# YukeWang96/QGTC_PPoPP22

Measured on AMD Instinct MI355X. Metric: effective bit-GEMM TOPS (2*M*K*N/t), 1-bit A x 1-bit X, M=K=4096, N=64, higher is better.
Workload: dtype fp4 (E2M1 codes of bit planes on MFMA, exact f32 sums); 1 GPU; bitMM2Bit 4096x4096x64 a=1 w=1 ob=1 (BASELINE.json configs[1], 2_7c shape); inputs=seeded Bernoulli(0.5) adjacency, uniform w-bit features, packed, resident in HBM, parallelism=replica-per-GPU x1, no data-path collective, engine=auto, issue=eager

## Files before the change

qgtc_ppopp22_amd/csrc/bitmm_fp4_one.hip.h:

```cpp
#pragma once

namespace {

constexpr int ONE_WAVES = 8;
constexpr int ONE_MAX_K = 4 * 128 * ONE_WAVES;

template <int NP>
__device__ __forceinline__ void one_expand(const u32x4 (&pl)[NP], int digit, uint32_t (&ops)[4][4], int (&scale)[4]) {
    if constexpr (NP == 1) {
#pragma unroll
        for (int t = 0; t < 4; t++) {
            const uint32_t wd = pl[0][t];
            ops[0][t] = wd & 0x11111111u;
            ops[1][t] = wd & 0x22222222u;
            ops[2][t] = wd & 0x44444444u;
            ops[3][t] = (wd >> 3) & 0x11111111u;
        }
        scale[0] = 128; scale[1] = 127; scale[2] = 126; scale[3] = 128;
    } else {
#pragma unroll
        for (int t = 0; t < 4; t++) {
            const uint32_t w0 = pl[2 * digit][t], w1 = 2 * digit + 1 < NP ? pl[(2 * digit + 1) % NP][t] : 0u;
            uint32_t ev = (w0 & 0x55555555u) | ((w1 & 0x55555555u) << 1), od = ((w0 >> 1) & 0x55555555u) | (w1 & 0xaaaaaaaau);
            asm("" : "+v"(ev), "+v"(od));
            ops[0][t] = ev & 0x33333333u;
            ops[1][t] = od & 0x33333333u;
            ops[2][t] = (ev >> 2) & 0x33333333u;
            ops[3][t] = (od >> 2) & 0x33333333u;
        }
#pragma unroll
        for (int s = 0; s < 4; s++) scale[s] = 128 + 2 * digit;
    }
}

template <int NA, int NW, int MODE, int RF, int CF>
__global__ __launch_bounds__(64 * ONE_WAVES) void k_bitmm_fp4_one(
    const uint32_t *__restrict__ Xp, const uint32_t *__restrict__ Wp, void *__restrict__ outp, uint32_t x_bytes,
    uint32_t w_bytes, uint32_t out_bytes, int M, int K, int N, int w_lines,
    uint32_t cfg ) {
    static_assert(NA >= 1 && NA <= 8 && NW >= 1 && NW <= 8, "plane capacities");
    static_assert(MODE != 1 || RF == 2, "cols-layout words need whole 32-row tiles");
    constexpr int NF = RF * CF;
    constexpr int NDA = (NA + 1) / 2, NDW = (NW + 1) / 2;
    constexpr bool SWAP = MODE != 1;
    __shared__ __attribute__((aligned(16))) f32x4 part[ONE_WAVES][NF][64];
    const int tid = threadIdx.x, lane = tid & 63;
    const int wv = __builtin_amdgcn_readfirstlane(tid >> 6);
    const int li = lane & 15, g = lane >> 4;
    const int kq = (K + 127) >> 7;
    const int m0 = blockIdx.x * (16 * RF), n0 = blockIdx.y * (16 * CF);
    const int a = cfg & 255u, w = (cfg >> 8) & 255u, ob = (cfg >> 16) & 255u;
    const bool zero_skip = ((cfg >> 24) & 1u) != 0u;
    const int nwv = min(ONE_WAVES, (kq + 3) >> 2);
    const bool worker = 4 * wv < kq;

#ifdef QGTC_STAMPS
    unsigned long long st_[8] = {0, 0, 0, 0, 0, 0, 0, 0};
#define ONE_STAMP(i) st_[i] = __builtin_amdgcn_s_memtime()
#else
#define ONE_STAMP(i) do { } while (0)
#endif
    ONE_STAMP(0);
    f32x4 acc[RF][CF];
    u32x4 xr[RF][NA], wr[CF][NW];
    {
        const uint32_t row_bytes = static_cast<uint32_t>(kq) * 16u;
        const int q = 4 * wv + g;
        const uint32_t ko = static_cast<uint32_t>(q) * 16u;
        const bool q_ok = q < kq;
        const __amdgpu_buffer_rsrc_t rx = __builtin_amdgcn_make_buffer_rsrc(const_cast<uint32_t *>(Xp), 0, static_cast<int>(x_bytes), 0x00020000);
        const __amdgpu_buffer_rsrc_t rw = __builtin_amdgcn_make_buffer_rsrc(const_cast<uint32_t *>(Wp), 0, static_cast<int>(w_bytes), 0x00020000);
        const uint32_t x_plane = static_cast<uint32_t>(pad8(M)) * row_bytes, w_plane = static_cast<uint32_t>(w_lines) * row_bytes;
#pragma unroll
        for (int i = 0; i < RF; i++) {
            const int m = m0 + 16 * i + li;
            uint32_t off = __umul24(static_cast<uint32_t>(m), row_bytes) + ko;
#ifdef QGTC_ABL
            if (cfg & (1u << 28)) off = static_cast<uint32_t>(lane) * 16u;
#endif
#pragma unroll
            for (int p = 0; p < NA; p++)
                xr[i][p] = __builtin_amdgcn_raw_buffer_load_b128(rx, (q_ok && m < M && p < a) ? off + static_cast<uint32_t>(p) * x_plane : 0xffffffffu, 0, 0);
        }
#pragma unroll
        for (int j = 0; j < CF; j++) {
            const int n = n0 + 16 * j + li;
            uint32_t off = __umul24(static_cast<uint32_t>(n), row_bytes) + ko;
#ifdef QGTC_ABL
            if (cfg & (1u << 29)) off = static_cast<uint32_t>(lane) * 16u;
#endif
#pragma unroll
            for (int p = 0; p < NW; p++)
                wr[j][p] = __builtin_amdgcn_raw_buffer_load_b128(rw, (q_ok && n < N && p < w) ? off + static_cast<uint32_t>(p) * w_plane : 0xffffffffu, 0, 0);
        }
    }
    if (worker) {
        ONE_STAMP(1);
        uint32_t any = 0u;
#pragma unroll
        for (int i = 0; i < RF; i++)
#pragma unroll
            for (int p = 0; p < NA; p++) any |= (xr[i][p].x | xr[i][p].y) | (xr[i][p].z | xr[i][p].w);
        const bool mult = !zero_skip || __ballot(any != 0u) != 0ull;
        if (!mult) {
#pragma unroll
            for (int i = 0; i < RF; i++)
#pragma unroll
                for (int j = 0; j < CF; j++) acc[i][j] = f32x4{0.0f, 0.0f, 0.0f, 0.0f};
        } else {
#ifdef QGTC_STAGGER_EXP
            if ((cfg & (1u << 30)) && wv >= 4) __builtin_amdgcn_s_sleep(6);
            if ((cfg & (1u << 31))) { if (wv >= 4) __builtin_amdgcn_s_setprio(0); else __builtin_amdgcn_s_setprio(2); }
            if ((cfg & (1u << 27)) && wv >= 4) __builtin_amdgcn_s_sleep(12);
#endif
            uint32_t xo[RF][NDA][4][4], wo[4][4];
            int xs[RF][NDA][4], ws[4];
#pragma unroll
            for (int i = 0; i < RF; i++)
#pragma unroll
                for (int da = 0; da < NDA; da++) one_expand<NA>(xr[i], da, xo[i][da], xs[i][da]);
#pragma unroll
            for (int j = 0; j < CF; j++)
#pragma unroll
                for (int dw = 0; dw < NDW; dw++) {
                    one_expand<NW>(wr[j], dw, wo, ws);
#pragma unroll
                    for (int s = 0; s < 4; s++) {
                        const i32x4 b4 = {static_cast<int>(wo[s][0]), static_cast<int>(wo[s][1]), static_cast<int>(wo[s][2]), static_cast<int>(wo[s][3])};
                        const i32x8 b8 = __builtin_shufflevector(b4, b4, 0, 1, 2, 3, -1, -1, -1, -1);
#pragma unroll
                        for (int i = 0; i < RF; i++)
#pragma unroll
                            for (int da = 0; da < NDA; da++) {
                                const i32x4 a4 = {static_cast<int>(xo[i][da][s][0]), static_cast<int>(xo[i][da][s][1]), static_cast<int>(xo[i][da][s][2]), static_cast<int>(xo[i][da][s][3])};
                                const i32x8 a8 = __builtin_shufflevector(a4, a4, 0, 1, 2, 3, -1, -1, -1, -1);
                                const f32x4 c = (dw == 0 && s == 0 && da == 0) ? f32x4{0.0f, 0.0f, 0.0f, 0.0f} : acc[i][j];
                                if (SWAP) acc[i][j] = __builtin_amdgcn_mfma_scale_f32_16x16x128_f8f6f4(b8, a8, c, 4, 4, 0, ws[s], 0, xs[i][da][s]);
                                else acc[i][j] = __builtin_amdgcn_mfma_scale_f32_16x16x128_f8f6f4(a8, b8, c, 4, 4, 0, xs[i][da][s], 0, ws[s]);
                            }
                    }
                }
        }
#ifdef QGTC_STAMPS
        asm volatile("" : "+v"(acc[0][0]));
#endif
        ONE_STAMP(2);
#pragma unroll
        for (int i = 0; i < RF; i++)
#pragma unroll
            for (int j = 0; j < CF; j++) part[wv][i * CF + j][lane] = acc[i][j];
    }
    int n_valid = 0;
    uint32_t vnib = 0u, oplane_bytes = 0u, o_off = 0xffffffffu, sh = 0u;
    bool store = false;
    const __amdgpu_buffer_rsrc_t ro = __builtin_amdgcn_make_buffer_rsrc(outp, 0, static_cast<int>(out_bytes), 0x00020000);
    if (wv < NF) {
        const int fi = wv / CF, fj = wv % CF;
        const int line = (SWAP ? m0 + 16 * fi : n0 + 16 * fj) + li;
        const int elem0 = (SWAP ? n0 + 16 * fj : m0 + 16 * fi) + 4 * g;
        const int line_lim = SWAP ? M : N, elem_lim = SWAP ? N : M;
        n_valid = line < line_lim ? min(max(elem_lim - elem0, 0), 4) : 0;
        vnib = (0xf0u >> n_valid) & 0xfu;
        const int pitch = SWAP ? step128(N) * 4 : step128(M) * 4;
        const int n_lines = SWAP ? pad8(M) : pad128(N);
        oplane_bytes = static_cast<uint32_t>(n_lines) * static_cast<uint32_t>(pitch) * 4u;
        const int frag0 = SWAP ? n0 + 16 * fj : m0 + 16 * fi;
        const int word = frag0 >> 5;
        o_off = MODE == 2 ? (static_cast<uint32_t>(line) * static_cast<uint32_t>(N) + static_cast<uint32_t>(elem0)) * 4u
                          : (static_cast<uint32_t>(line) * static_cast<uint32_t>(pitch) + static_cast<uint32_t>(word)) * 4u + ((frag0 & 16) ? 0u : 2u);
        store = MODE == 2 ? line < M : (g == 0 && line < n_lines && word < pitch);
        if (!store) o_off = 0xffffffffu;
        sh = 12u - 4u * static_cast<uint32_t>(g);
        asm volatile("" : "+v"(o_off) : "v"(vnib), "v"(sh), "s"(oplane_bytes));
    }
    ONE_STAMP(3);
    __syncthreads();
    ONE_STAMP(4);

    if (wv >= NF) {
        uint32_t *out = static_cast<uint32_t *>(outp);
        const int t = tid - 64 * NF, nt = 64 * (ONE_WAVES - NF);
        if (MODE == 0) {
            const int rows_pad = pad8(M), row_words = step128(N) * 4;
            const int w_next = (n0 + 16 * CF + 31) >> 5;
            if (static_cast<int>(blockIdx.y) == (N + 16 * CF - 1) / (16 * CF) - 1 && w_next < row_words) {
                const int nx = row_words - w_next;
                for (int e = t; e < ob * 16 * RF * nx; e += nt) {
                    const int x = e % nx, r = (e / nx) % (16 * RF), p = e / (nx * 16 * RF);
                    if (m0 + r < rows_pad) out[(static_cast<size_t>(p) * rows_pad + m0 + r) * row_words + w_next + x] = 0u;
                }
            }
        } else if (MODE == 1) {
            const int lines = pad128(N), line_words = step128(M) * 4;
            const size_t oplane = static_cast<size_t>(lines) * line_words;
            const bool last_m = static_cast<int>(blockIdx.x) == (M + 16 * RF - 1) / (16 * RF) - 1, last_n = static_cast<int>(blockIdx.y) == (N + 16 * CF - 1) / (16 * CF) - 1;
            const int word1 = m0 >> 5, w_core1 = min(line_words, word1 + 1);
            if (last_m && w_core1 < line_words) {
                for (int e = t; e < ob * 16 * CF; e += nt) {
                    const int line = n0 + e % (16 * CF), p = e / (16 * CF);
                    if (line < lines)
                        for (int wi = w_core1; wi < line_words; wi++) out[p * oplane + static_cast<size_t>(line) * line_words + wi] = 0u;
                }
            }
            if (last_n && n0 + 16 * CF < lines) {
                const int nl = lines - (n0 + 16 * CF), w_end = last_m ? line_words : w_core1;
                for (int e = t; e < ob * nl; e += nt) {
                    const int line = n0 + 16 * CF + e % nl, p = e / nl;
                    for (int wi = word1; wi < w_end; wi++) out[p * oplane + static_cast<size_t>(line) * line_words + wi] = 0u;
                }
            }
        }
        return;
    }

    f32x4 sum;
    if (nwv == ONE_WAVES) {
        f32x4 pv[ONE_WAVES];
#ifdef QGTC_ABL_HALFRED
#pragma unroll
        for (int p = 0; p < ONE_WAVES / 2; p++) pv[p] = part[p][wv][lane];
        sum = (pv[0] + pv[1]) + (pv[2] + pv[3]);
#else
#pragma unroll
        for (int p = 0; p < ONE_WAVES; p++) pv[p] = part[p][wv][lane];
        sum = ((pv[0] + pv[1]) + (pv[2] + pv[3])) + ((pv[4] + pv[5]) + (pv[6] + pv[7]));
#endif
    } else {
        sum = part[0][wv][lane];
        for (int p = 1; p < nwv; p++) sum += part[p][wv][lane];
    }
    ONE_STAMP(5);
    if (MODE == 2) {
        const u32x4 v4 = __builtin_bit_cast(u32x4, sum);
        if (n_valid == 4) {
            __builtin_amdgcn_raw_buffer_store_b128(v4, ro, o_off, 0, 0);
        } else {
            if (n_valid >= 2) __builtin_amdgcn_raw_buffer_store_b64(u32x2{v4.x, v4.y}, ro, o_off, 0, 0);
            if (n_valid == 3) __builtin_amdgcn_raw_buffer_store_b32(v4.z, ro, o_off + 8u, 0, 0);
            if (n_valid == 1) __builtin_amdgcn_raw_buffer_store_b32(v4.x, ro, o_off, 0, 0);
        }
    } else {
        const int maxi = 1 << ob;
        uint32_t P = 0u;
#pragma unroll
        for (int e = 0; e < 4; e++) {
            const int c = static_cast<int>(sum[e]);
            P = (P << 8) | (static_cast<uint32_t>(c > maxi ? maxi - 1 : c) & 255u);
        }
        int qhi[4];
        if (ob > 8) {
#pragma unroll
            for (int e = 0; e < 4; e++) {
                const int c = static_cast<int>(sum[e]);
                qhi[e] = c > maxi ? maxi - 1 : c;
            }
        }
        for (int p = 0; p < ob; p++, o_off += store ? oplane_bytes : 0u) {
            uint32_t t;
            if (p < 8) t = (P >> p) & 0x01010101u;
            else t = ((qhi[0] >> p) & 1) << 24 | ((qhi[1] >> p) & 1) << 16 | ((qhi[2] >> p) & 1) << 8 | ((qhi[3] >> p) & 1);
            uint32_t x = (((t >> 21) | (t >> 14)) | ((t >> 7) | t)) & vnib;
            x <<= sh;
            const auto s16 = __builtin_amdgcn_permlane16_swap(x, x, false, false);
            x = s16[0] | s16[1];
            x = or_with_partner_half(x);
            __builtin_amdgcn_raw_buffer_store_b16(static_cast<unsigned short>(x), ro, o_off, 0, 0);
        }
    }
#ifdef QGTC_STAMPS
    ONE_STAMP(6);
    if (tid == 0 && blockIdx.y == 0 && blockIdx.x < 1024)
        for (int i = 0; i < 8; i++) g_stamps[blockIdx.x * 16 + i] = st_[i];
#endif
#undef ONE_STAMP
}

}
```

Baseline: 738.2 TOPS.

## Simplify load addressing, move pad zeroing into output waves, early-exit idle waves

Load offsets are now built from a per-lane base plus wave-uniform scalar terms, and the per-row bounds checks on X/W loads are dropped, so address math is cheaper. The zero-skip path writes zeros straight into the shared partials, and the accumulator is scoped to the multiply branch. Non-output waves now sync and return earlier. MODE 0 padding zeroing moves from the idle waves into the output waves as per-lane b32 stores placed beside the reduction loads. The cost is that correctness now depends on padded rows (M, N) staying in bounds, and MODE 0 padding now rides on the store waves.

Result: slower. 632.1 TOPS (-14.4%).

```diff
diff --git a/qgtc_ppopp22_amd/csrc/bitmm_fp4_one.hip.h b/qgtc_ppopp22_amd/csrc/bitmm_fp4_one.hip.h
--- a/qgtc_ppopp22_amd/csrc/bitmm_fp4_one.hip.h
+++ b/qgtc_ppopp22_amd/csrc/bitmm_fp4_one.hip.h
@@ -61,37 +61,37 @@
 #define ONE_STAMP(i) do { } while (0)
 #endif
     ONE_STAMP(0);
-    f32x4 acc[RF][CF];
     u32x4 xr[RF][NA], wr[CF][NW];
     {
         const uint32_t row_bytes = static_cast<uint32_t>(kq) * 16u;
-        const int q = 4 * wv + g;
-        const uint32_t ko = static_cast<uint32_t>(q) * 16u;
-        const bool q_ok = q < kq;
+        const uint32_t lo = __umul24(static_cast<uint32_t>(li), row_bytes) + static_cast<uint32_t>(g) * 16u;
+        const bool q_ok = (lane & 48) < 16 * (kq - 4 * wv);
         const __amdgpu_buffer_rsrc_t rx = __builtin_amdgcn_make_buffer_rsrc(const_cast<uint32_t *>(Xp), 0, static_cast<int>(x_bytes), 0x00020000);
         const __amdgpu_buffer_rsrc_t rw = __builtin_amdgcn_make_buffer_rsrc(const_cast<uint32_t *>(Wp), 0, static_cast<int>(w_bytes), 0x00020000);
         const uint32_t x_plane = static_cast<uint32_t>(pad8(M)) * row_bytes, w_plane = static_cast<uint32_t>(w_lines) * row_bytes;
+        const uint32_t ux = static_cast<uint32_t>(m0) * row_bytes + 64u * static_cast<uint32_t>(wv);
+        const uint32_t uw = static_cast<uint32_t>(n0) * row_bytes + 64u * static_cast<uint32_t>(wv);
 #pragma unroll
         for (int i = 0; i < RF; i++) {
-            const int m = m0 + 16 * i + li;
-            uint32_t off = __umul24(static_cast<uint32_t>(m), row_bytes) + ko;
+#pragma unroll
+            for (int p = 0; p < NA; p++) {
+                uint32_t off = lo + (ux + static_cast<uint32_t>(16 * i) * row_bytes + static_cast<uint32_t>(p) * x_plane);
 #ifdef QGTC_ABL
-            if (cfg & (1u << 28)) off = static_cast<uint32_t>(lane) * 16u;
-#endif
-#pragma unroll
-            for (int p = 0; p < NA; p++)
-                xr[i][p] = __builtin_amdgcn_raw_buffer_load_b128(rx, (q_ok && m < M && p < a) ? off + static_cast<uint32_t>(p) * x_plane : 0xffffffffu, 0, 0);
+                if (cfg & (1u << 28)) off = static_cast<uint32_t>(lane) * 16u;
+#endif
+                xr[i][p] = __builtin_amdgcn_raw_buffer_load_b128(rx, (q_ok && (p == 0 || p < a)) ? off : 0xffffffffu, 0, 0);
+            }
         }
 #pragma unroll
         for (int j = 0; j < CF; j++) {
-            const int n = n0 + 16 * j + li;
-            uint32_t off = __umul24(static_cast<uint32_t>(n), row_bytes) + ko;
+#pragma unroll
+            for (int p = 0; p < NW; p++) {
+                uint32_t off = lo + (uw + static_cast<uint32_t>(16 * j) * row_bytes + static_cast<uint32_t>(p) * w_plane);
 #ifdef QGTC_ABL
-            if (cfg & (1u << 29)) off = static_cast<uint32_t>(lane) * 16u;
-#endif
-#pragma unroll
-            for (int p = 0; p < NW; p++)
-                wr[j][p] = __builtin_amdgcn_raw_buffer_load_b128(rw, (q_ok && n < N && p < w) ? off + static_cast<uint32_t>(p) * w_plane : 0xffffffffu, 0, 0);
+                if (cfg & (1u << 29)) off = static_cast<uint32_t>(lane) * 16u;
+#endif
+                wr[j][p] = __builtin_amdgcn_raw_buffer_load_b128(rw, (p == 0 || p < w) ? off : 0xffffffffu, 0, 0);
+            }
         }
     }
     if (worker) {
@@ -102,12 +102,14 @@
 #pragma unroll
             for (int p = 0; p < NA; p++) any |= (xr[i][p].x | xr[i][p].y) | (xr[i][p].z | xr[i][p].w);
         const bool mult = !zero_skip || __ballot(any != 0u) != 0ull;
-        if (!mult) {
-#pragma unroll
-            for (int i = 0; i < RF; i++)
-#pragma unroll
-                for (int j = 0; j < CF; j++) acc[i][j] = f32x4{0.0f, 0.0f, 0.0f, 0.0f};
+        if (__builtin_expect(!mult, 0)) {
+            f32x4 z = {0.0f, 0.0f, 0.0f, 0.0f};
+            asm volatile("" : "+v"(z));
+#pragma unroll
+            for (int f = 0; f < NF; f++) part[wv][f][lane] = z;
+            asm volatile("" ::: "memory");
         } else {
+            f32x4 acc[RF][CF];
 #ifdef QGTC_STAGGER_EXP
             if ((cfg & (1u << 30)) && wv >= 4) __builtin_amdgcn_s_sleep(6);
             if ((cfg & (1u << 31))) { if (wv >= 4) __builtin_amdgcn_s_setprio(0); else __builtin_amdgcn_s_setprio(2); }
@@ -140,21 +142,50 @@
                             }
                     }
                 }
-        }
 #ifdef QGTC_STAMPS
-        asm volatile("" : "+v"(acc[0][0]));
-#endif
-        ONE_STAMP(2);
-#pragma unroll
-        for (int i = 0; i < RF; i++)
-#pragma unroll
-            for (int j = 0; j < CF; j++) part[wv][i * CF + j][lane] = acc[i][j];
-    }
-    int n_valid = 0;
-    uint32_t vnib = 0u, oplane_bytes = 0u, o_off = 0xffffffffu, sh = 0u;
-    bool store = false;
+            asm volatile("" : "+v"(acc[0][0]));
+#endif
+            ONE_STAMP(2);
+#pragma unroll
+            for (int i = 0; i < RF; i++)
+#pragma unroll
+                for (int j = 0; j < CF; j++) part[wv][i * CF + j][lane] = acc[i][j];
+        }
+    }
+    if (wv >= NF) {
+        __syncthreads();
+        if (MODE == 1) {
+            uint32_t *out = static_cast<uint32_t *>(outp);
+            const int t = tid - 64 * NF, nt = 64 * (ONE_WAVES - NF);
+            const int lines = pad128(N), line_words = step128(M) * 4;
+            const size_t oplane = static_cast<size_t>(lines) * line_words;
+            const bool last_m = static_cast<int>(blockIdx.x) == (M + 16 * RF - 1) / (16 * RF) - 1, last_n = static_cast<int>(blockIdx.y) == (N + 16 * CF - 1) / (16 * CF) - 1;
+            const int word1 = m0 >> 5, w_core1 = min(line_words, word1 + 1);
+            if (last_m && w_core1 < line_words) {
+                for (int l = t; l < 16 * CF; l += nt) {
+                    const int line = n0 + l;
+                    if (line < lines)
+                        for (int p = 0; p < ob; p++)
+                            for (int wi = w_core1; wi < line_words; wi++) out[p * oplane + static_cast<size_t>(line) * line_words + wi] = 0u;
+                }
+            }
+            if (last_n && n0 + 16 * CF < lines) {
+                const int nl = lines - (n0 + 16 * CF), w_end = last_m ? line_words : w_core1;
+                for (int l = t; l < nl; l += nt) {
+                    const int line = n0 + 16 * CF + l;
+                    for (int p = 0; p < ob; p++)
+                        for (int wi = word1; wi < w_end; wi++) out[p * oplane + static_cast<size_t>(line) * line_words + wi] = 0u;
+                }
+            }
+        }
+        return;
+    }
+
     const __amdgpu_buffer_rsrc_t ro = __builtin_amdgcn_make_buffer_rsrc(outp, 0, static_cast<int>(out_bytes), 0x00020000);
-    if (wv < NF) {
+    int n_valid;
+    uint32_t vnib, oplane_bytes, o_off, o_step, sh, p_off = 0xffffffffu, p_step = 0u, pad_wave = 0u;
+    bool store;
+    {
         const int fi = wv / CF, fj = wv % CF;
         const int line = (SWAP ? m0 + 16 * fi : n0 + 16 * fj) + li;
         const int elem0 = (SWAP ? n0 + 16 * fj : m0 + 16 * fi) + 4 * g;
@@ -171,62 +202,41 @@
         store = MODE == 2 ? line < M : (g == 0 && line < n_lines && word < pitch);
         if (!store) o_off = 0xffffffffu;
         sh = 12u - 4u * static_cast<uint32_t>(g);
-        asm volatile("" : "+v"(o_off) : "v"(vnib), "v"(sh), "s"(oplane_bytes));
+        if (MODE == 0) {
+            const int w_next = (n0 + 16 * CF + 31) >> 5, nx = pitch - w_next;
+            pad_wave = (fj == 0 && static_cast<int>(blockIdx.y) == (N + 16 * CF - 1) / (16 * CF) - 1 && nx > 0) ? 1u : 0u;
+            const bool pad = pad_wave != 0u && g >= 1 && g <= nx && line < n_lines;
+            p_off = pad ? (static_cast<uint32_t>(line) * static_cast<uint32_t>(pitch) + static_cast<uint32_t>(w_next + g - 1)) * 4u : 0xffffffffu;
+            p_step = pad ? oplane_bytes : 0u;
+        }
+        o_step = store ? oplane_bytes : 0u;
+        asm volatile("" : "+v"(o_off), "+v"(p_off) : "v"(vnib), "v"(sh), "v"(o_step), "v"(p_step));
     }
     ONE_STAMP(3);
     __syncthreads();
     ONE_STAMP(4);
 
-    if (wv >= NF) {
-        uint32_t *out = static_cast<uint32_t *>(outp);
-        const int t = tid - 64 * NF, nt = 64 * (ONE_WAVES - NF);
-        if (MODE == 0) {
-            const int rows_pad = pad8(M), row_words = step128(N) * 4;
-            const int w_next = (n0 + 16 * CF + 31) >> 5;
-            if (static_cast<int>(blockIdx.y) == (N + 16 * CF - 1) / (16 * CF) - 1 && w_next < row_words) {
-                const int nx = row_words - w_next;
-                for (int e = t; e < ob * 16 * RF * nx; e += nt) {
-                    const int x = e % nx, r = (e / nx) % (16 * RF), p = e / (nx * 16 * RF);
-                    if (m0 + r < rows_pad) out[(static_cast<size_t>(p) * rows_pad + m0 + r) * row_words + w_next + x] = 0u;
-                }
-            }
-        } else if (MODE == 1) {
-            const int lines = pad128(N), line_words = step128(M) * 4;
-            const size_t oplane = static_cast<size_t>(lines) * line_words;
-            const bool last_m = static_cast<int>(blockIdx.x) == (M + 16 * RF - 1) / (16 * RF) - 1, last_n = static_cast<int>(blockIdx.y) == (N + 16 * CF - 1) / (16 * CF) - 1;
-            const int word1 = m0 >> 5, w_core1 = min(line_words, word1 + 1);
-            if (last_m && w_core1 < line_words) {
-                for (int e = t; e < ob * 16 * CF; e += nt) {
-                    const int line = n0 + e % (16 * CF), p = e / (16 * CF);
-                    if (line < lines)
-                        for (int wi = w_core1; wi < line_words; wi++) out[p * oplane + static_cast<size_t>(line) * line_words + wi] = 0u;
-                }
-            }
-            if (last_n && n0 + 16 * CF < lines) {
-                const int nl = lines - (n0 + 16 * CF), w_end = last_m ? line_words : w_core1;
-                for (int e = t; e < ob * nl; e += nt) {
-                    const int line = n0 + 16 * CF + e % nl, p = e / nl;
-                    for (int wi = word1; wi < w_end; wi++) out[p * oplane + static_cast<size_t>(line) * line_words + wi] = 0u;
-                }
-            }
-        }
-        return;
-    }
-
     f32x4 sum;
+    const auto pad_stores = [&]() {
+        if (MODE == 0 && pad_wave != 0u)
+            for (int p = 0; p < ob; p++, p_off += p_step) __builtin_amdgcn_raw_buffer_store_b32(0u, ro, p_off, 0, 0);
+    };
     if (nwv == ONE_WAVES) {
         f32x4 pv[ONE_WAVES];
 #ifdef QGTC_ABL_HALFRED
 #pragma unroll
         for (int p = 0; p < ONE_WAVES / 2; p++) pv[p] = part[p][wv][lane];
+        pad_stores();
         sum = (pv[0] + pv[1]) + (pv[2] + pv[3]);
 #else
 #pragma unroll
         for (int p = 0; p < ONE_WAVES; p++) pv[p] = part[p][wv][lane];
+        pad_stores();
         sum = ((pv[0] + pv[1]) + (pv[2] + pv[3])) + ((pv[4] + pv[5]) + (pv[6] + pv[7]));
 #endif
     } else {
         sum = part[0][wv][lane];
+        pad_stores();
         for (int p = 1; p < nwv; p++) sum += part[p][wv][lane];
     }
     ONE_STAMP(5);
@@ -255,7 +265,7 @@
                 qhi[e] = c > maxi ? maxi - 1 : c;
             }
         }
-        for (int p = 0; p < ob; p++, o_off += store ? oplane_bytes : 0u) {
+        for (int p = 0; p < ob; p++, o_off += o_step) {
             uint32_t t;
             if (p < 8) t = (P >> p) & 0x01010101u;
             else t = ((qhi[0] >> p) & 1) << 24 | ((qhi[1] >> p) & 1) << 16 | ((qhi[2] >> p) & 1) << 8 | ((qhi[3] >> p) & 1);
```
